# lazytiger/pbrt-rs

Hardware: AMD Instinct MI355X
Metric: Mrays/s (higher is better)
Workload: dtype f32

## Files before the change

pbrt-rs_amd/csrc/kernel_select.h:

```cpp
#pragma once
#include <type_traits>

#include "scene.h"
#include "trace_wide.h"

namespace pb {

enum class TraceKind { Stackless, Wide, Shapes, Spheres, Binary, Moving };
struct TraceChoice {
    TraceKind kind;
    int inst;
    bool count;
    bool ok;
};

inline TraceChoice choose_trace(const PbrtHipScene* s) {
    const PbrtHipContext* ctx = s->ctx;
    TraceChoice c{TraceKind::Binary, s->d.bvh.instanced ? (s->d.bvh.general_top ? 2 : 1) : 0, ctx->count_traversal == 1, true};
    if (ctx->traversal == PBRT_TRAVERSAL_STACKLESS) {
        c.kind = TraceKind::Stackless;
        c.ok = stackless_applies(s);
    } else if (s->has_wide && ctx->count_traversal != 1 && ctx->traversal == PBRT_TRAVERSAL_AUTO) {
        c.kind = TraceKind::Wide;
        c.count = ctx->count_traversal == 2;
// ... 78 lines not shown
                                               {k_shade_direct<D, 3>, k_shade_direct<W, 3>},
                                               {k_shade_direct<D, 2>, k_shade_direct<W, 2>},
                                               {k_shade_direct<D, 1>, k_shade_direct<W, 1>},
                                               {k_shade_direct<D, 0>, k_shade_direct<W, 0>}};
    static constexpr DirectKernel ao[2] = {k_shade_direct<AO, kDirectShapes>, k_shade_direct<AO, 0>};
    if (n.moving) return moving_direct_kernel(integrator);
    if (n.lobes && (integrator == D || integrator == W)) return lobe_direct_kernel(integrator == W);
    if (integrator == D || integrator == W) return lit[n.column()][integrator == W];
    return ao[n.shapes ? 0 : 1];
}

inline PathKernel path_kernel(const SceneNeeds& n, bool bin) {
    static constexpr PathKernel table[2][6] = {
        {k_shade_shapes<true>, k_shade_maps<true>, k_shade<true, 3>, k_shade<true, 2>, k_shade<true, 1>, k_shade<true, 0>},
        {k_shade_shapes<false>, k_shade_maps<false>, k_shade<false, 3>, k_shade<false, 2>, k_shade<false, 1>, k_shade<false, 0>}};
    if (n.moving) return moving_path_kernel(bin);
    if (n.lobes) return lobe_path_kernel(bin);
    return table[bin ? 0 : 1][n.column()];
}

inline DirectKernel lobe_direct_kernel(bool whitted) {
    static constexpr DirectKernel table[2] = {k_shade_direct<PBRT_INTEGRATOR_DIRECT, 3 + kDirectLobes>,
                                              k_shade_direct<PBRT_INTEGRATOR_WHITTED, 3 + kDirectLobes>};
    return table[whitted ? 1 : 0];
}
inline PathKernel lobe_path_kernel(bool bin) {
    static constexpr PathKernel table[2] = {k_shade_lobes<true>, k_shade_lobes<false>};
    return table[bin ? 0 : 1];
}

inline DirectKernel moving_direct_kernel(int integrator) {
    static constexpr DirectKernel table[3] = {k_shade_direct<PBRT_INTEGRATOR_DIRECT, 3 + kDirectMoving>,
                                              k_shade_direct<PBRT_INTEGRATOR_WHITTED, 3 + kDirectMoving>,
                                              k_shade_direct<PBRT_INTEGRATOR_AO, kDirectMoving>};
    return table[integrator == PBRT_INTEGRATOR_DIRECT ? 0 : integrator == PBRT_INTEGRATOR_WHITTED ? 1 : 2];
}
inline PathKernel moving_path_kernel(bool bin) {
    static constexpr PathKernel table[2] = {k_shade_moving<true>, k_shade_moving<false>};
    return table[bin ? 0 : 1];
}

using GenerateKernel = void (*)(PathState, Queues, PassParams, DevCamera, TileList);
using GenerateCameraKernel = void (*)(PathState, Queues, PassParams, DevCamera, DevMotion, TileList);
constexpr int kGenerateCameraAnimated = 2;
inline int generate_key(bool scene_moving, bool camera_animated) { return (scene_moving ? 1 : 0) | (camera_animated ? kGenerateCameraAnimated : 0); }
inline GenerateKernel generate_kernel(int key) {
    static constexpr GenerateKernel table[2] = {k_generate, k_generate_moving};
    return table[key & 1];
}
inline GenerateCameraKernel generate_camera_kernel(int key) {
    static constexpr GenerateCameraKernel table[2] = {k_generate_moving_camera, k_generate_moving_camera};
    return table[key & 1];
}
#endif

}
```

pbrt-rs_amd/csrc/render.hip:

```cpp
#include <hip/hip_runtime.h>
#include "abi_guard.h"

#include <algorithm>
#include <chrono>
#include <cstdio>
#include <cstdlib>
#include <cstring>
#include <string>
#include <thread>
#include <vector>

#include "host_motion.h"
#include "scene.h"
#include "trace.h"
#include "wavefront.h"
#define PB_SELECT_SHADING_KERNELS
#include "kernel_select.h"

using namespace pb;

static int camera_row(PbrtHipContext* ctx, const PbrtCamera& camera, const PbrtCameraMotion* motion, DevMotion* storage,
                      const DevMotion** row) {
    *row = nullptr;
    if (!motion || !motion->animated) return PBRT_HIP_OK;
// ... 777 lines not shown
        return hip_ok(ctx, hipEventCreate(&begin), "hipEventCreate") && hip_ok(ctx, hipEventCreate(&end), "hipEventCreate") &&
               hip_ok(ctx, hipEventCreate(&t0), "hipEventCreate") && hip_ok(ctx, hipEventCreate(&t1), "hipEventCreate");
    }
    ~RenderEvents() {
        for (hipEvent_t e : {begin, end, t0, t1})
            if (e) (void)hipEventDestroy(e);
    }
};

struct SortBufs {
    uint32_t *keys[2] = {nullptr, nullptr}, *vals = nullptr;
    void* tmp = nullptr;
    size_t tmp_bytes = 0;
};

constexpr int kSortFrom = 2;

struct RenderJob {
    PbrtHipScene* s;
    PbrtHipContext* ctx;
    hipStream_t st;
    const LiBatch* li;
    float* d_film;
    const DevMotion* camera_motion;
    PbrtRenderParams rp;
    bool li_mode, export_mode;
    bool tabulated;
    bool direct;
    bool box;
    float frx, fry;
    int32_t sb[4];
    int world, rank;
    int n_pix = 0, spp_pass = 0;
    int64_t valid_pixels = 0;
    size_t N = 0;
    PathState ps;
    Queues q[2];
    bool sort_rays = false, sort_shade = false, bin_shade = false;
    SortBufs ray_sort;
    SortBufs shade_sort;
    uint32_t* shade_positions = nullptr;
    TraceChoice trace;
    uint32_t* special_list = nullptr;
    std::vector<int> prefix;
    SamplerParams smp{};
    DirectState ds{};
    float* d_filter = nullptr;
    float4* accum = nullptr;
    TileList tiles{};
    DevCamera cam;
    ShadeConsts sc;
    DirectKernel shade_direct = nullptr;
    PathKernel shade_path[2] = {nullptr, nullptr};
    PbrtRenderStats local{};

    int invalid(const char* m) const {
        ctx->last_error = m;
        return PBRT_HIP_ERR_INVALID;
    }
    int round_count(int n) const { return rp.sampler == PBRT_SAMPLER_ZEROTWO ? round_up_pow2(n) : n; }
    const char* normalise_params(const PbrtRenderParams& rp_in);
    int size_pass();
    int alloc_path_buffers(DevBuf& buf, bool* ok);
    int setup_sampler(DevBuf& buf, bool* ok);
    int setup_light_distribution(const SceneNeeds& needs);
    PassParams pass_params(int s0) const;
    void wait_for_counts(int& rc);
    void trace_wavefront(const RenderEvents& ev, const Queues& qcur, uint32_t n_trace, int wavefront, int& rc);
    void shade_wavefront(const PassParams& pp, int cur, int nxt, uint32_t n_shade, int wavefront, int& rc);
    void run_wavefronts(const RenderEvents& ev, const PassParams& pp, uint32_t n_paths, int& rc);
    void film_stage(const PassParams& pp, uint32_t n_paths, bool last_pass, int& rc);
    int run(const PbrtCamera& camera, PbrtRenderStats* stats);
};

const char* RenderJob::normalise_params(const PbrtRenderParams& rp_in) {
    rp = rp_in;
    li_mode = li && li->d_rays;
    export_mode = li && li->out_rays;
    if (li_mode) {
        if (li->n <= 0 || li->n > (1ll << 28)) return "li: batch size must be in [1, 2^28]";
        rp.width = (int32_t)li->n;
        rp.height = 1;
        rp.spp = 1;
        rp.x0 = rp.y0 = 0;
        rp.x1 = rp.width;
        rp.y1 = 1;
        rp.tile_rank = 0;
        rp.tile_world = 1;
        rp.spp_per_pass = 1;
        rp.sampler = PBRT_SAMPLER_RANDOM;
        rp.filter_table = nullptr;
    }
    if (rp.width <= 0 || rp.height <= 0 || rp.spp <= 0) return "width, height and spp must be positive";
    if (rp.sampler < PBRT_SAMPLER_RANDOM || rp.sampler > PBRT_SAMPLER_HALTON) return "unknown sampler";
    tabulated = rp.sampler != PBRT_SAMPLER_RANDOM;
    if (tabulated && (rp.sampler_dims < 0 || rp.sampler_dims > 63)) return "sampler_dims must be in [0, 63]";
    if (const char* why = sampler_spp(rp, &rp.spp)) return why;
    if (rp.integrator == PBRT_INTEGRATOR_AO && rp.ao_samples >= 1 && rp.ao_samples <= 65535 && tabulated)
        rp.ao_samples = round_count(rp.ao_samples);
    frx = rp.filter_radius[0] > 0.0f ? rp.filter_radius[0] : 0.5f;
    fry = rp.filter_radius[1] > 0.0f ? rp.filter_radius[1] : 0.5f;
    box = true;
    if (rp.filter_table) {
        if (frx != 0.5f || fry != 0.5f) box = false;
        for (int i = 0; i < 256; ++i)
            if (rp.filter_table[i] != 1.0f) box = false;
// ... 204 lines not shown
    pp.n_pix = n_pix;
    pp.n_samples = std::min(spp_pass, rp.spp - s0);
    const int want = rp.samples_per_wave > 0 ? rp.samples_per_wave : ((tabulated && rp.sampler != PBRT_SAMPLER_HALTON) ? 1 : 64);
    pp.group_shift = 0;
    while ((2 << pp.group_shift) <= want && pp.group_shift < 6 && pp.n_samples % (2 << pp.group_shift) == 0) ++pp.group_shift;
    if (li_mode || export_mode) pp.group_shift = 0;
    pp.sample0 = s0;
    pp.spp = rp.spp;
    pp.width = rp.width;
    pp.height = rp.height;
    pp.x0 = rp.x0;
    pp.y0 = rp.y0;
    pp.x1 = rp.x1;
    pp.y1 = rp.y1;
    pp.sb_x0 = sb[0];
    pp.sb_y0 = sb[1];
    pp.sb_w = sb[2] - sb[0];
    pp.seed = rp.seed;
    pp.max_depth = rp.max_depth;
    pp.rr_threshold = rp.rr_threshold;
    pp.light_strategy = rp.light_strategy;
    pp.filter_rx = frx;
    pp.filter_ry = fry;
    pp.filter_table = d_filter;
    pp.max_sample_luminance = rp.max_sample_luminance > 0.0f ? rp.max_sample_luminance : INFINITY;
    pp.stream_keys = li_mode ? li->d_keys : nullptr;
    return pp;
}

#define RENDER_TRY(call) \
    if (rc == PBRT_HIP_OK && !hip_ok(ctx, (call), #call)) rc = PBRT_HIP_ERR_DEVICE;

void RenderJob::wait_for_counts(int& rc) {
    hipError_t qe;
    const auto spin_start = std::chrono::steady_clock::now();
    uint32_t polls = 0;
    while ((qe = hipEventQuery(ctx->ev_sync)) == hipErrorNotReady) {
        if ((++polls & 0xfffu) == 0) {
            const double waited = std::chrono::duration<double>(std::chrono::steady_clock::now() - spin_start).count();
            if (waited > ctx->wavefront_deadline_s) {
                ctx->last_error = "a wavefront did not finish within the deadline (hung kernel?)";
                ctx->lost = true;
                rc = PBRT_HIP_ERR_DEVICE;
                break;
            }
            if (waited > 0.05) std::this_thread::yield();
        }
    }
    if (rc == PBRT_HIP_OK) RENDER_TRY(qe);
}

void RenderJob::trace_wavefront(const RenderEvents& ev, const Queues& qcur, uint32_t n_trace, int wavefront, int& rc) {
    RENDER_TRY(hipMemsetAsync(ctx->d_work_counter, 0, kWorkCounters * sizeof(unsigned int), st));
    const uint32_t* trace_queue = qcur.trace;
    if (sort_rays && wavefront >= kSortFrom && n_trace >= (1u << 20)) {
        const SortBufs& rs = ray_sort;
        size_t tb = rs.tmp_bytes;
        if (pb::sort_pairs_u32(st, rs.tmp, &tb, rs.keys[0], rs.keys[1], qcur.trace, rs.vals, n_trace, kSortKeyBits) != 0 && rc == PBRT_HIP_OK) {
            ctx->last_error = "rocPRIM radix sort failed";
            rc = PBRT_HIP_ERR_DEVICE;
        }
        trace_queue = rs.vals;
    }
    RENDER_TRY(hipEventRecord(ev.t0, st));
    const int segments = (wavefront == 0 && !trace.inst) ? kQueueSegments : 1;
    dispatch(trace, [&](auto kind, auto count, auto inst) {
        constexpr TraceKind K = decltype(kind)::value;
        constexpr bool COUNT = decltype(count)::value;
        constexpr int INST = decltype(inst)::value;
        const dim3 grid(persistent_grid(s)), block(kTraceBlock);
        if constexpr (K == TraceKind::Stackless) {
            hipLaunchKernelGGL(k_trace_stackless, dim3(stackless_grid(s)), block, 0, st, s->d.bvh, ps, trace_queue, n_trace, ctx->d_work_counter,
                               segments);
        } else if constexpr (K == TraceKind::Wide) {
            WideTrees wt = s->wide;
            wt.special_list = special_list;
            wt.special_count = ctx->d_work_counter + kSpecialCount;
            hipLaunchKernelGGL((k_trace_wide<COUNT, INST>), dim3(wide_grid<COUNT, INST>(s)), block, 0, st, wt, ps, trace_queue, n_trace,
                               ctx->d_work_counter, segments, ctx->d_counters);
            hipLaunchKernelGGL(k_trace_special<INST>, grid, block, 0, st, s->d.bvh, ps, trace_queue, n_trace, special_list,
                               ctx->d_work_counter + kSpecialCount, ctx->d_work_counter + kFollowUpCounter);
        } else if constexpr (K == TraceKind::Shapes) {
            hipLaunchKernelGGL(k_trace_shapes<COUNT>, grid, block, 0, st, s->d.bvh, ps, trace_queue, n_trace, ctx->d_work_counter, ctx->d_counters,
                               segments);
        } else if constexpr (K == TraceKind::Moving) {
            hipLaunchKernelGGL((k_trace_moving<COUNT, INST>), dim3(persistent_grid(s, PB_MOVING_TRACE_WAVES)), block, 0, st, s->d.bvh, s->d_motions, ps,
                               trace_queue, n_trace, ctx->d_work_counter, ctx->d_counters, segments);
        } else {
            hipLaunchKernelGGL((k_trace<COUNT, INST, K == TraceKind::Spheres>), grid, block, 0, st, s->d.bvh, ps, trace_queue, n_trace,
                               ctx->d_work_counter, ctx->d_counters, segments);
        }
    });
    RENDER_TRY(hipGetLastError());
    RENDER_TRY(hipEventRecord(ev.t1, st));
}

void RenderJob::shade_wavefront(const PassParams& pp, int cur, int nxt, uint32_t n_shade, int wavefront, int& rc) {
    const dim3 grid((n_shade + 255) / 256), block(256);
    if (direct) {
        hipLaunchKernelGGL(shade_direct, grid, block, 0, st, sc, ps, ds, q[cur], q[nxt], pp, tiles, n_shade);
        return;
    }
    const Queues qin = q[cur];
    const uint32_t* order = nullptr;
    if (sort_shade && wavefront >= 1 && n_shade >= (1u << 10)) {
        const SortBufs& ss = shade_sort;
        hipLaunchKernelGGL(k_shade_sort_keys, dim3((n_shade + 255) / 256), dim3(256), 0, st, sc, ps, q[cur].shade, n_shade, pp.max_depth,
                           ss.keys[0], shade_positions);
        size_t tb = ss.tmp_bytes;
        if (pb::sort_pairs_u32(st, ss.tmp, &tb, ss.keys[0], ss.keys[1], shade_positions, ss.vals, n_shade, (s->bxdfs || s->disney || s->lobes) ? 4 : 3) != 0 &&
            rc == PBRT_HIP_OK) {
            ctx->last_error = "rocPRIM radix sort failed";
            rc = PBRT_HIP_ERR_DEVICE;
        }
        order = ss.vals;
    }
    hipLaunchKernelGGL(shade_path[bin_shade && wavefront >= 1], grid, block, 0, st, sc, ps, qin, q[nxt], pp, tiles, n_shade, order);
    std::swap(ps.ray, ps.ray_next);
    std::swap(ps.nee_a, ps.nee_a_next);
    std::swap(ps.nee_f, ps.nee_f_next);
    std::swap(ps.nee_b, ps.nee_b_next);
    std::swap(ps.nee_light, ps.nee_light_next);
}

void RenderJob::run_wavefronts(const RenderEvents& ev, const PassParams& pp, uint32_t n_paths, int& rc) {
    unsigned long long counts[2] = {n_paths, n_paths};
    local.camera_samples += (uint64_t)valid_pixels * pp.n_samples;
    local.rays_closest += (uint64_t)valid_pixels * pp.n_samples;
    int cur = 0, wavefront = 0;
    while (rc == PBRT_HIP_OK && counts[1] > 0) {
        uint32_t n_trace = (uint32_t)counts[0], n_shade = (uint32_t)counts[1];
        if (n_trace > 0) trace_wavefront(ev, q[cur], n_trace, wavefront, rc);
        int nxt = cur ^ 1;
        RENDER_TRY(hipMemsetAsync(q[nxt].counts64, 0, 2 * sizeof(unsigned long long), st));
        q[nxt].keys = (sort_rays && wavefront + 1 >= kSortFrom) ? ray_sort.keys[0] : nullptr;
        shade_wavefront(pp, cur, nxt, n_shade, wavefront, rc);
        RENDER_TRY(hipGetLastError());
        RENDER_TRY(hipMemcpyAsync(ctx->h_counts, q[nxt].counts64, sizeof(counts), hipMemcpyDeviceToHost, st));
        RENDER_TRY(hipEventRecord(ctx->ev_sync, st));
        if (rc == PBRT_HIP_OK) wait_for_counts(rc);
        counts[0] = ctx->h_counts[0];
        counts[1] = ctx->h_counts[1];
        if (n_trace > 0 && rc == PBRT_HIP_OK) {
            float ms = 0.0f;
            RENDER_TRY(hipEventElapsedTime(&ms, ev.t0, ev.t1));
            local.trace_ms += ms;
            local.trace_launches += 1;
            if (ctx->trace_log)
                std::fprintf(stderr, "[pbrt_hip] k_trace: %u rays %.3f ms (%.0f Mrays/s), k_shade: %u paths\n", n_trace, ms, n_trace / ms * 1e-3,
                             n_shade);
            ctx->trace_ms += ms;
            ctx->trace_launches += 1;
        }
        const uint64_t n_rays = counts[0] & 0xffffffffull, n_shadow = counts[0] >> 32;
        local.rays_closest += n_rays - n_shadow;
        local.rays_shadow += n_shadow;
        counts[0] = n_rays;
        wavefront += 1;
        cur = nxt;
    }
}

void RenderJob::film_stage(const PassParams& pp, uint32_t n_paths, bool last_pass, int& rc) {
    if (li_mode) {
        hipLaunchKernelGGL(k_li_output, dim3((unsigned)((li->n + 255) / 256)), dim3(256), 0, st, ps, (uint32_t)li->n, li->d_rgb);
        RENDER_TRY(hipGetLastError());
        return;
    }
    if (!box) {
        hipLaunchKernelGGL(k_film_splat, dim3((n_paths + 255) / 256), dim3(256), 0, st, ps, pp, tiles, d_film);
// ... 35 lines not shown
        valid_pixels += (int64_t)(std::min(o.x + kTile, rp.x1) - o.x) * (std::min(o.y + kTile, rp.y1) - o.y);
    if (li_mode) valid_pixels = li->n;
    if (int rc = size_pass()) return rc;
    if (export_mode && spp_pass != rp.spp) return invalid("camera rays: too many samples for one pass");
    N = (size_t)n_pix * spp_pass;
    if (N * 4 >= (1ull << 32)) return invalid("too many concurrent paths for 32-bit queue entries; lower spp_per_pass");

    DevBuf buf(ctx);
    bool ok = true;
    if (int rc = alloc_path_buffers(buf, &ok)) return rc;
    if (int rc = setup_sampler(buf, &ok)) return rc;
    int* d_prefix = buf.alloc<int>(prefix.size(), &ok);
    if (direct) {
        ds.stage = buf.alloc<int>(N, &ok);
        ds.ld_acc = buf.alloc<float4>(N, &ok);
        ds.frames = buf.alloc<float4>(N * (size_t)std::max(1, rp.max_depth) * 3, &ok);
        ds.light_strategy = rp.light_strategy;
        ds.mode = rp.integrator;
        ds.ao_samples = rp.ao_samples;
        ds.ao_cos_sample = rp.light_strategy != 0;
        if (prefix.back() >= 0xfff0) return invalid("too many light samples per vertex");
    }
    if (!box) {
        d_filter = buf.alloc<float>(256, &ok);
        if (ok) HIP_TRY(ctx, hipMemcpyAsync(d_filter, rp.filter_table, 256 * sizeof(float), hipMemcpyHostToDevice, st));
    }
    accum = buf.alloc<float4>(n_pix, &ok);
    int2* d_origins = buf.alloc<int2>(origins.size(), &ok);
    if (!ok) return PBRT_HIP_ERR_OOM;
    HIP_TRY(ctx, hipMemcpyAsync(d_origins, origins.data(), origins.size() * sizeof(int2), hipMemcpyHostToDevice, st));
    HIP_TRY(ctx, hipMemsetAsync(accum, 0, (size_t)n_pix * sizeof(float4), st));
    HIP_TRY(ctx, hipMemcpyAsync(d_prefix, prefix.data(), prefix.size() * sizeof(int), hipMemcpyHostToDevice, st));
    tiles = TileList{d_origins, (int)origins.size()};

    std::memcpy(cam.c2w, camera.camera_to_world, 64);
    std::memcpy(cam.r2c, camera.raster_to_camera, 64);
    cam.lens_radius = camera.lens_radius;
    cam.focal_distance = camera.focal_distance;
    cam.shutter_open = camera.shutter_open;
    cam.shutter_close = camera.shutter_close;
    cam.kind = camera.kind;
    if (camera.kind < PBRT_CAMERA_PERSPECTIVE || camera.kind > PBRT_CAMERA_ENVIRONMENT) return invalid("unknown camera kind");

    const SceneNeeds needs = scene_needs(s);
    scene_shade_consts(s, &sc);
    sc.light_sample_prefix = d_prefix;
    sc.total_light_samples = prefix.back();
    if (int rc = setup_light_distribution(needs)) return rc;
    if (direct) {
        shade_direct = direct_kernel(needs, rp.integrator);
    } else {
        shade_path[0] = path_kernel(needs, false);
        shade_path[1] = path_kernel(needs, true);
    }

    RenderEvents ev;
    if (!ev.create(ctx)) return PBRT_HIP_ERR_DEVICE;
    int rc = PBRT_HIP_OK;
    RENDER_TRY(hipEventRecord(ev.begin, st));
    bool tables_ready = !tabulated || rp.sampler == PBRT_SAMPLER_HALTON;
    for (int s0 = 0; s0 < rp.spp && rc == PBRT_HIP_OK; s0 += spp_pass) {
        const PassParams pp = pass_params(s0);
        const uint32_t n_paths = (uint32_t)n_pix * pp.n_samples;
        if (!tables_ready) {
            hipLaunchKernelGGL(k_sampler_tables, dim3((n_pix + 63) / 64), dim3(64), 0, st, pp, tiles);
            RENDER_TRY(hipGetLastError());
            tables_ready = true;
        }
        if (li_mode)
            hipLaunchKernelGGL(k_li_generate, dim3((n_paths + 255) / 256), dim3(256), 0, st, ps, q[0], li->d_rays, li->d_keys, (uint32_t)li->n,
                               n_paths, li->skip);
        else if (const int key = generate_key(s->moving, camera_motion != nullptr); key & kGenerateCameraAnimated)
            hipLaunchKernelGGL(generate_camera_kernel(key), dim3((n_paths + 255) / 256), dim3(256), 0, st, ps, q[0], pp, cam, *camera_motion, tiles);
        else
            hipLaunchKernelGGL(generate_kernel(key), dim3((n_paths + 255) / 256), dim3(256), 0, st, ps, q[0], pp, cam, tiles);
        RENDER_TRY(hipGetLastError());
        if (export_mode) {
            hipLaunchKernelGGL(k_camera_rays_out, dim3((n_paths + 255) / 256), dim3(256), 0, st, ps, pp, tiles, li->out_rays, li->out_keys,
                               li->out_pfilm, li->out_pixel_sample);
            RENDER_TRY(hipGetLastError());
            break;
        }
        if (direct) {
            RENDER_TRY(hipMemsetAsync(ds.stage, 0, (size_t)n_paths * sizeof(int), st));
            RENDER_TRY(hipMemsetAsync(ds.ld_acc, 0, (size_t)n_paths * sizeof(float4), st));
        }
        run_wavefronts(ev, pp, n_paths, rc);
        film_stage(pp, n_paths, s0 + spp_pass >= rp.spp, rc);
    }
    RENDER_TRY(hipEventRecord(ev.end, st));
    if (!ctx->lost) {
        const hipError_t drained = hipStreamSynchronize(st);
        if (rc == PBRT_HIP_OK && !hip_ok(ctx, drained, "hipStreamSynchronize (end of render)")) rc = PBRT_HIP_ERR_DEVICE;
    }
    if (rc == PBRT_HIP_OK) {
        float ms = 0.0f;
        RENDER_TRY(hipEventElapsedTime(&ms, ev.begin, ev.end));
        local.total_ms = ms;
    }
    if (stats) *stats = local;
    return rc;
}
}

int wavefront_render(PbrtHipScene* s, const PbrtCamera& camera, const PbrtRenderParams& rp_in, float* d_film,
                     PbrtRenderStats* stats, const LiBatch* li, const DevMotion* camera_motion) {
    RenderJob job{s, s->ctx, s->ctx->stream, li, d_film, camera_motion};
    if (const char* why = job.normalise_params(rp_in)) return job.invalid(why);
    return job.run(camera, stats);
}
#undef RENDER_TRY

#ifdef PB_LANE_STATS
extern "C" int pbrt_hip_debug_wide_stats(unsigned long long* out24, int reset) try {
    if (hipMemcpyFromSymbol(out24, HIP_SYMBOL(pb::g_wide_stats), 32 * sizeof(unsigned long long)) != hipSuccess) return 1;
    if (reset) {
        unsigned long long z[32] = {0};
        if (hipMemcpyToSymbol(HIP_SYMBOL(pb::g_wide_stats), z, sizeof(z)) != hipSuccess) return 1;
    }
    return 0;
}
PB_ABI_CATCH
extern "C" int pbrt_hip_debug_lane_stats(unsigned long long* out8, int reset) try {
    if (hipMemcpyFromSymbol(out8, HIP_SYMBOL(pb::g_lane_stats), 8 * sizeof(unsigned long long)) != hipSuccess) return 1;
    if (reset) {
        unsigned long long z[8] = {0, 0, 0, 0, 0, 0, 0, 0};
        if (hipMemcpyToSymbol(HIP_SYMBOL(pb::g_lane_stats), z, sizeof(z)) != hipSuccess) return 1;
    }
// ... 5 lines not shown
```

pbrt-rs_amd/csrc/wavefront.h:

```cpp
#pragma once
#include <hip/hip_runtime.h>

#include "wf_state.h"
#include "wf_sampler.h"
#include "wf_generate_trace.h"
#include "wf_surface.h"
#include "wf_lights.h"
#include "wf_lobes.h"
#include "wf_path.h"
#include "wf_direct.h"
#include "wf_film.h"
#include "wf_camera_motion.h"

struct LiBatch {
    const PbrtRay* d_rays = nullptr;
    const uint64_t* d_keys = nullptr;
    int64_t n = 0;
    int skip = 0;
    float* d_rgb = nullptr;
    PbrtRay* out_rays = nullptr;
    uint64_t* out_keys = nullptr;
    float* out_pfilm = nullptr;
    int32_t* out_pixel_sample = nullptr;
};
int wavefront_render(PbrtHipScene* s, const PbrtCamera& camera, const PbrtRenderParams& rp, float* d_film,
                     PbrtRenderStats* stats, const LiBatch* li = nullptr, const pb::DevMotion* camera_motion = nullptr);
```

pbrt-rs_amd/csrc/wf_generate_trace.h:

```cpp
#pragma once
#include "wf_sampler.h"

namespace pb {

PB_DEV void camera_rows_at(const DevCamera& cam, const DevMotion& mo, float time, float* rows) {
    if (time <= mo.start_time) {
        for (int k = 0; k < 12; ++k) rows[k] = cam.c2w[k];
    } else if (time >= mo.end_time) {
        for (int k = 0; k < 12; ++k) rows[k] = mo.end_o2w[k];
    } else {
        motion_interpolate_forward(mo, time, rows);
    }
}
PB_DEV V3 xform_point_rows(const float* m, V3 p) {
    return V3{m[0] * p.x + m[1] * p.y + m[2] * p.z + m[3], m[4] * p.x + m[5] * p.y + m[6] * p.z + m[7],
              m[8] * p.x + m[9] * p.y + m[10] * p.z + m[11]};
}

template <bool TIME, bool CAMERA_MOTION = false>
PB_DEV void generate_camera_rays(const PathState& ps, const Queues& q, const PassParams& pp, const DevCamera& cam, const TileList& tiles,
                                 const DevMotion* cmo = nullptr) {
    uint32_t p = blockIdx.x * blockDim.x + threadIdx.x;
    uint32_t n = (uint32_t)pp.n_pix * pp.n_samples;
    if (p >= n) return;
    int s_local, pix;
    path_to_sample_pixel(pp, p, &s_local, &pix);
    int tile = pix >> 8, within = pix & 255;
    int2 org = tiles.origin[tile];
    int x = org.x + (within & 15), y = org.y + (within >> 4);
    bool valid = x >= pp.x0 && x < pp.x1 && y >= pp.y0 && y < pp.y1;
    int flags = 0;
    if (valid) {
        int s = pp.sample0 + s_local;
        Samp sm;
        rng_set_sequence(sm.rng, sample_sequence(pp, x, y, s));
        sm.pix = pix;
        sm.s = s;
        sm.dim1 = sm.dim2 = sm.arr = 0;
        sm.h_offset = pp.smp.kind == PBRT_SAMPLER_HALTON ? halton_pixel_offset(pp.smp, x, y) : 0;
        float u0, u1, l0, l1;
        samp_2d(pp, sm, &u0, &u1);
        float pfx = (float)x + u0, pfy = (float)y + u1;
        float time_u = samp_1d(pp, sm);
        samp_2d(pp, sm, &l0, &l1);
        V3 o = V3{0.0f, 0.0f, 0.0f}, d;
        if (cam.kind == PBRT_CAMERA_ENVIRONMENT) {
            float theta = kPi * pfy / (float)pp.height;
            float phi = 2.0f * kPi * pfx / (float)pp.width;
            float st, ct, sp, cp;
            det_sincos(theta, &st, &ct);
            det_sincos(phi, &sp, &cp);
            d = V3{st * cp, ct, st * sp};
        } else if (cam.kind == PBRT_CAMERA_ORTHOGRAPHIC) {
            o = xform_point(cam.r2c, V3{pfx, pfy, 0.0f});
            d = V3{0.0f, 0.0f, 1.0f};
            if (cam.lens_radius > 0.0f) {
                float lx, ly;
                concentric_sample_disk(l0, l1, &lx, &ly);
                lx *= cam.lens_radius;
                ly *= cam.lens_radius;
                float ft = cam.focal_distance / d.z;
                V3 p_focus = o + d * ft;
                o.x += lx;
                o.y += ly;
                d = normalize(p_focus - o);
            }
        } else {
            V3 p_camera = xform_point(cam.r2c, V3{pfx, pfy, 0.0f});
            d = normalize(p_camera);
            if (cam.lens_radius > 0.0f) {
                float lx, ly;
                concentric_sample_disk(l0, l1, &lx, &ly);
                lx *= cam.lens_radius;
                ly *= cam.lens_radius;
                float ft = cam.focal_distance / d.z;
                V3 p_focus = o + d * ft;
                o = V3{lx, ly, 0.0f};
                d = normalize(p_focus - o);
            }
        }
        (void)time_u;
        const float* m = cam.c2w;
        float rows[12], time = 0.0f;
        if (CAMERA_MOTION) {
            time = (1.0f - time_u) * cam.shutter_open + time_u * cam.shutter_close;
            camera_rows_at(cam, *cmo, time, rows);
            m = rows;
        }
        V3 ow = CAMERA_MOTION ? xform_point_rows(m, o) : xform_point(m, o);
        float xa = __builtin_fabsf(m[0] * o.x) + __builtin_fabsf(m[1] * o.y) + __builtin_fabsf(m[2] * o.z) + __builtin_fabsf(m[3]);
        float ya = __builtin_fabsf(m[4] * o.x) + __builtin_fabsf(m[5] * o.y) + __builtin_fabsf(m[6] * o.z) + __builtin_fabsf(m[7]);
        float za = __builtin_fabsf(m[8] * o.x) + __builtin_fabsf(m[9] * o.y) + __builtin_fabsf(m[10] * o.z) + __builtin_fabsf(m[11]);
        V3 o_err = V3{xa, ya, za} * kGamma3;
        V3 dw = xform_vector(m, d);
        float l2 = len2(dw);
        float tmax = kInf;
        if (l2 > 0.0f) {
            float dt = dot(vabs(dw), o_err) / l2;
            ow = ow + dw * dt;
            tmax -= dt;
        }
        store_ray(ps, p, RS_CONT, ow, dw, tmax);
        if (CAMERA_MOTION)
            ps.ray[ray_index(ps, p, RS_CONT) + 1].w = time;
        else if (TIME)
            ps.ray[ray_index(ps, p, RS_CONT) + 1].w = (1.0f - time_u) * cam.shutter_open + time_u * cam.shutter_close;
        samp_store(ps, p, sm);
        ps.pfilm[p] = make_float2(pfx, pfy);
        flags = PF_VALID | PF_ALIVE;
    } else {
        ps.pfilm[p] = make_float2(0.0f, 0.0f);
    }
    ps.L[p] = make_float4(0.0f, 0.0f, 0.0f, 1.0f);
    ps.beta[p] = make_float4(1.0f, 1.0f, 1.0f, __int_as_float(flags));
    if (!valid) store_ray(ps, p, RS_CONT, V3{0.0f, 0.0f, 0.0f}, V3{0.0f, 0.0f, 1.0f}, -1.0f);
    q.trace[p] = p * 4u + RS_CONT;
    q.shade[p] = p;
}
__global__ void k_generate(PathState ps, Queues q, PassParams pp, DevCamera cam, TileList tiles) {
    generate_camera_rays<false>(ps, q, pp, cam, tiles);
}

__global__ void k_li_generate(PathState ps, Queues q, const PbrtRay* __restrict__ rays, const uint64_t* __restrict__ keys, uint32_t n,
                              uint32_t n_padded, int skip) {
    uint32_t p = blockIdx.x * blockDim.x + threadIdx.x;
    if (p >= n_padded) return;
    int flags = 0;
    if (p < n) {
        Rng rng;
        rng_set_sequence(rng, keys[p]);
        for (int k = 0; k < skip; ++k) (void)rng_u32(rng);
        ps.rng[p] = rng.state;
        ps.samp[p] = 0;
        const float4* rp = reinterpret_cast<const float4*>(rays + p);
        float4 a = rp[0], b = rp[1];
        store_ray(ps, p, RS_CONT, V3{a.x, a.y, a.z}, V3{a.w, b.x, b.y}, b.z);
        ps.ray[ray_index(ps, p, RS_CONT) + 1].w = b.w;
        flags = PF_VALID | PF_ALIVE;
    } else {
        store_ray(ps, p, RS_CONT, V3{0.0f, 0.0f, 0.0f}, V3{0.0f, 0.0f, 1.0f}, -1.0f);
    }
    ps.pfilm[p] = make_float2(0.0f, 0.0f);
    ps.L[p] = make_float4(0.0f, 0.0f, 0.0f, 1.0f);
    ps.beta[p] = make_float4(1.0f, 1.0f, 1.0f, __int_as_float(flags));
    q.trace[p] = p * 4u + RS_CONT;
    q.shade[p] = p;
}
__global__ void k_li_output(PathState ps, uint32_t n, float* __restrict__ rgb) {
    uint32_t p = blockIdx.x * blockDim.x + threadIdx.x;
    if (p >= n) return;
    float4 L = ps.L[p];
    rgb[3 * (size_t)p] = L.x;
    rgb[3 * (size_t)p + 1] = L.y;
    rgb[3 * (size_t)p + 2] = L.z;
}
__global__ void k_camera_rays_out(PathState ps, PassParams pp, TileList tiles, PbrtRay* __restrict__ rays, uint64_t* __restrict__ keys,
                                  float* __restrict__ pfilm, int32_t* __restrict__ pixel_sample) {
    uint32_t p = blockIdx.x * blockDim.x + threadIdx.x;
    uint32_t n = (uint32_t)pp.n_pix * pp.n_samples;
    if (p >= n) return;
    int s_local, pix;
    path_to_sample_pixel(pp, p, &s_local, &pix);
    int2 org = tiles.origin[pix >> 8];
    int x = org.x + (pix & 15), y = org.y + ((pix & 255) >> 4);
    bool valid = (__float_as_int(ps.beta[p].w) & PF_VALID) != 0;
    size_t ri = ray_index(ps, p, RS_CONT);
    float4 a = ps.ray[ri], b = ps.ray[ri + 1];
    float4* out = reinterpret_cast<float4*>(rays + p);
    out[0] = a;
    out[1] = b;
    keys[p] = sample_sequence(pp, x, y, pp.sample0 + s_local);
    float2 pf = ps.pfilm[p];
    pfilm[2 * (size_t)p] = pf.x;
    pfilm[2 * (size_t)p + 1] = pf.y;
    pixel_sample[3 * (size_t)p] = valid ? x : -1;
    pixel_sample[3 * (size_t)p + 1] = valid ? y : -1;
    pixel_sample[3 * (size_t)p + 2] = pp.sample0 + s_local;
}

template <bool TWO_LEVEL>
struct WavefrontRayIO {
    PathState ps;
    const uint32_t* __restrict__ queue;
    uint32_t count;
    int n_segments;
    PB_DEV uint32_t n() const { return count; }
    PB_DEV int segments() const { return n_segments; }
    PB_DEV uint32_t token(uint32_t i) const { return queue[i]; }
    PB_DEV bool strict(uint32_t e) const { return (e & 3u) == RS_MIS_BOOL; }
    PB_DEV bool load(uint32_t e, TravRay* r, bool* any) const {
        uint32_t p = e >> 2, slot = e & 3u;
        size_t ri = ray_index(ps, p, slot == RS_MIS_BOOL ? (uint32_t)RS_MIS : slot);
        float4 a = ps.ray[ri], b = ps.ray[ri + 1];
        *r = TravRay{a.x, a.y, a.z, a.w, b.x, b.y, b.z};
        *any = slot >= RS_SHADOW;
        return !(b.z < 0.0f);
    }
    PB_DEV bool load(uint32_t e, TravRay* r, bool* any, float* time) const {
        uint32_t p = e >> 2, slot = e & 3u;
        size_t ri = ray_index(ps, p, slot == RS_MIS_BOOL ? (uint32_t)RS_MIS : slot);
        float4 a = ps.ray[ri], b = ps.ray[ri + 1];
        *r = TravRay{a.x, a.y, a.z, a.w, b.x, b.y, b.z};
        *any = slot >= RS_SHADOW;
        *time = b.w;
        return !(b.z < 0.0f);
    }
    PB_DEV void store(uint32_t e, bool any, bool found, float t, float b0, float b1, float b2, int slot, int inst) const {
        uint32_t p = e >> 2, rs = e & 3u;
        if (rs == RS_MIS_BOOL) {
            ps.hit[hit_index(ps, p, RS_MIS)] = make_float4(__int_as_float(found ? 0 : -1), 0.0f, 0.0f, 0.0f);
            return;
        }
        size_t ri = hit_index(ps, p, rs);
        if (any) {
            ps.hit[ri] = make_float4(found ? 1.0f : 0.0f, 0.0f, 0.0f, 0.0f);
        } else {
            (void)t;
            ps.hit[ri] = make_float4(__int_as_float(found ? slot : -1), b0, b1, b2);
            if (TWO_LEVEL) ps.hit[ri + 1] = make_float4(__int_as_float(inst), 0.0f, 0.0f, 0.0f);
        }
    }
};

template <bool COUNT, int INST, bool SPH = false>
__global__ void __launch_bounds__(kTraceBlock, (COUNT || SPH) ? 4 : (INST ? PB_INST_WAVES : PB_TRACE_WAVES))
    k_trace(DevBVH bvh, PathState ps, const uint32_t* __restrict__ queue, uint32_t n, unsigned int* work_counter,
            unsigned long long* counters, int segments) {
    __shared__ uint2 lds_stack[kStackLds * kTraceBlock];
    WavefrontRayIO<INST != 0> io{ps, queue, n, segments};
    trace_persistent<WavefrontRayIO<INST != 0>, COUNT, INST, SPH>(bvh, io, work_counter, lds_stack + threadIdx.x,
                                                  blockIdx.x * kTraceBlock + threadIdx.x, counters);
}

template <bool COUNT>
__global__ void __launch_bounds__(kTraceBlock, 4)
    k_trace_shapes(DevBVH bvh, PathState ps, const uint32_t* __restrict__ queue, uint32_t n, unsigned int* work_counter,
                   unsigned long long* counters, int segments) {
    __shared__ uint2 lds_stack[kStackLds * kTraceBlock];
    WavefrontRayIO<false> io{ps, queue, n, segments};
    trace_persistent<WavefrontRayIO<false>, COUNT, 0, false, true>(bvh, io, work_counter, lds_stack + threadIdx.x,
                                                                   blockIdx.x * kTraceBlock + threadIdx.x, counters);
// ... 47 lines not shown
```

pbrt-rs_amd/csrc/wf_path.h:

```cpp
#pragma once
#include "wf_lights.h"

namespace pb {

PB_DEV uint32_t shade_key(const ShadeConsts& sc, const PathState& ps, uint32_t p, uint32_t rec, int max_depth) {
    int fb = __float_as_int(ps.beta[p].w);
    uint32_t key = 0;
    if ((fb & PF_ALIVE) && (fb >> 8) < max_depth) {
        const size_t hb = hit_index(ps, rec, RS_CONT);
        int slot = __float_as_int(ps.hit[hb].x), inst = hit_instance(ps, hb);
        if (slot >= 0) {
            int mat = __float_as_int(sc.bvh.tris[3 * (size_t)slot + 2].z);
            if (sc.bvh.instanced && inst >= 0) {
                int over = __float_as_int(sc.bvh.instances[7 * (size_t)inst + 6].x);
                if (over >= 0) mat = over;
            }
            key = 1u + (uint32_t)sc.materials[mat].type;
        }
    }
    return key;
}
__global__ void k_shade_sort_keys(ShadeConsts sc, PathState ps, const uint32_t* __restrict__ shade_queue, uint32_t n, int max_depth,
                                  uint32_t* __restrict__ keys, uint32_t* __restrict__ positions) {
    uint32_t i = blockIdx.x * blockDim.x + threadIdx.x;
    if (i >= n) return;
    keys[i] = shade_key(sc, ps, shade_queue[i], i, max_depth);
    positions[i] = i;
}

constexpr int shade_keys(int level) { return level == 4 ? 13 : level == 3 ? 12 : level == 2 ? 11 : level == 1 ? 8 : 6; }
template <int KEYS>
struct ShadeBins {
    uint32_t count[4][KEYS];
    uint32_t path[256];
    uint32_t rec[256];
};

#ifndef PB_SHADE_WAVES
#define PB_SHADE_WAVES 3
#endif
template <bool BIN, int LEVEL, bool SHP, bool ML = false, bool MOV = false>
PB_DEV void shade_bounce(const ShadeConsts& sc, const PathState& ps, const Queues& qin, const Queues& qout, const PassParams& pp,
                         const TileList& tiles, uint32_t n_in, const uint32_t* __restrict__ order) {
    constexpr bool GLOSSY = LEVEL >= 1;
    constexpr bool LOBES = LEVEL == 4;
    constexpr int kShadeKeys = shade_keys(LEVEL);
    uint32_t i = blockIdx.x * blockDim.x + threadIdx.x;
    bool active = i < n_in;
    uint32_t rec = (active && order) ? order[i] : i;
    uint32_t p = active ? qin.shade[rec] : 0u;
    __shared__ StagedRecords staged;
    const StageSink stage{staged};
    if (BIN) {
        __shared__ ShadeBins<kShadeKeys> bins;
        const int lane = threadIdx.x & 63, wave = threadIdx.x >> 6;
        const uint32_t key = active ? shade_key(sc, ps, p, rec, pp.max_depth) : (uint32_t)(kShadeKeys - 1);
        uint32_t rank = 0;
#pragma unroll
        for (int k = 0; k < kShadeKeys; ++k) {
            const unsigned long long m = __ballot(key == (uint32_t)k);
            if (key == (uint32_t)k) rank = lane_prefix(m);
            if (lane == 0) bins.count[wave][k] = (uint32_t)__popcll(m);
        }
        __syncthreads();
        uint32_t before = 0;
        for (int k = 0; k < kShadeKeys; ++k)
            for (int w = 0; w < 4; ++w)
                before += ((uint32_t)k < key || ((uint32_t)k == key && w < wave)) ? bins.count[w][k] : 0u;
        bins.path[before + rank] = p;
        bins.rec[before + rank] = rec;
        uint32_t n_active = 0;
        for (int k = 0; k < kShadeKeys - 1; ++k)
            for (int w = 0; w < 4; ++w) n_active += bins.count[w][k];
        __syncthreads();
        p = bins.path[threadIdx.x];
        rec = bins.rec[threadIdx.x];
        active = threadIdx.x < n_active;
    }
    bool emit_cont = false, emit_mis = false, emit_shadow = false, mis_bool = false;

    uint32_t cell = 0;
    float time = 0.0f;
    if (active) {
        float4 Lq = ps.L[p], bq = ps.beta[p];
        V3 L = V3{Lq.x, Lq.y, Lq.z};
        float eta_scale = Lq.w;
        V3 beta = V3{bq.x, bq.y, bq.z};
        int fb = __float_as_int(bq.w);
        int flags = fb & 0xff, bounces = fb >> 8;
        size_t rbase = ray_index(ps, rec, RS_CONT), hbase = hit_index(ps, rec, RS_CONT);

        if (flags & (PF_NEE_SHADOW | PF_NEE_MIS)) {
            float pick_pdf;
            V3 beta_v;
            V3 ld = estimate_direct_resolve<SHP>(sc, ps, rec, flags, &pick_pdf, &beta_v);
            ld = ld / pick_pdf;
            L = L + mulv(beta_v, ld);
            flags &= ~(PF_NEE_SHADOW | PF_NEE_MIS);
        }

        if (flags & PF_ALIVE) {
            flags &= ~PF_ALIVE;
            float4 r0 = ps.ray[rbase], r1 = ps.ray[rbase + 1];
            V3 rd = V3{r0.w, r1.x, r1.y};
            float4 h0 = ps.hit[hbase];
            int hslot = __float_as_int(h0.x);
            bool found = hslot >= 0;
            Surf sf;
            if (MOV) time = r1.w;
            if (found) {
                if constexpr (MOV)
                    sf = surface_from_hit_moving(sc.bvh, sc.motions, time, hslot, hit_instance(ps, hbase), h0.y, h0.z, h0.w, rd);
                else
                    sf = surface_from_hit<SHP>(sc.bvh, hslot, hit_instance(ps, hbase), h0.y, h0.z, h0.w, rd);
                if (qout.keys) cell = ray_sort_cell(sf.p.x, sf.p.y, sf.p.z, qout.key_lo, qout.key_inv);
            }
            if (bounces == 0 || (flags & PF_SPECULAR_BOUNCE)) {
                if (found) {
                    L = L + mulv(beta, surface_le(sc, sf, -rd));
                } else {
                    for (int k = 0; k < sc.n_infinite; ++k) {
                        DevLight lt = sc.lights[sc.infinite_ids[k]];
                        V3 le = lt.slot >= 0 ? env_le(sc.env_maps[lt.slot], rd) : V3{lt.L[0], lt.L[1], lt.L[2]};
                        L = L + mulv(beta, le);
                    }
                }
            }
            if (found && bounces < pp.max_depth) {
                DevMaterial mat = sc.materials[sf.material];
                Samp sm = path_sampler(ps, pp, tiles, p);
                if (mat.type == PBRT_MAT_NONE) {
                    V3 o = offset_ray_origin(sf.p, sf.p_error, sf.n, rd);
                    stage.ray(RS_CONT, o, rd, kInf);
                    flags |= PF_ALIVE;
                    emit_cont = true;
                } else {
                    Frame fr = make_frame(sf);
                    V3 kd = V3{mat.kd[0], mat.kd[1], mat.kd[2]};
                    V3 kt = V3{mat.kt[0], mat.kt[1], mat.kt[2]};
                    V3 wo = -rd;
                    bool has_lobe;
                    bool nonspecular;
                    typename LevelBsdf<LEVEL>::type nsb;
                    if (GLOSSY) {
                        load_bsdf(sc, sf.material, mat, &nsb);
                        nonspecular = nsb.n > 0;
                        if (mat.type == PBRT_MAT_GLASS) has_lobe = !(is_black(kd) && is_black(kt));
                        else if (mat.type == PBRT_MAT_MIRROR) has_lobe = !is_black(kd);
                        else has_lobe = nonspecular;
                        if constexpr (LOBES)
                            if (nsb.row) has_lobe = nsb.row->n > 0;
                    } else {
                        if (mat.type == PBRT_MAT_GLASS) has_lobe = !(is_black(kd) && is_black(kt));
                        else has_lobe = !is_black(kd);
                        nonspecular = (mat.type == PBRT_MAT_MATTE) && has_lobe;
                    }
// ... 128 lines not shown
```

Measured before the change: 3026.

## Use implicit identity queues and initial path state for the first wavefront

```diff
diff --git a/pbrt-rs_amd/csrc/kernel_select.h b/pbrt-rs_amd/csrc/kernel_select.h
--- a/pbrt-rs_amd/csrc/kernel_select.h
+++ b/pbrt-rs_amd/csrc/kernel_select.h
@@ -154,6 +154,22 @@
     static constexpr GenerateCameraKernel table[2] = {k_generate_moving_camera, k_generate_moving_camera};
     return table[key & 1];
 }
+
+inline GenerateKernel implicit_generate_kernel(int key) {
+    static constexpr GenerateKernel table[2] = {k_generate_implicit, k_generate_moving_implicit};
+    return table[key & 1];
+}
+inline GenerateCameraKernel implicit_generate_camera_kernel(int key) {
+    static constexpr GenerateCameraKernel table[2] = {k_generate_moving_camera_implicit, k_generate_moving_camera_implicit};
+    return table[key & 1];
+}
+inline PathKernel first_path_kernel(const SceneNeeds& n) {
+    static constexpr PathKernel table[6] = {k_shade_shapes_first, k_shade_maps_first, k_shade_first<3>,
+                                            k_shade_first<2>,     k_shade_first<1>,   k_shade_first<0>};
+    if (n.moving) return k_shade_moving_first;
+    if (n.lobes) return k_shade_lobes_first;
+    return table[n.column()];
+}
 #endif
 
 }
diff --git a/pbrt-rs_amd/csrc/render.hip b/pbrt-rs_amd/csrc/render.hip
--- a/pbrt-rs_amd/csrc/render.hip
+++ b/pbrt-rs_amd/csrc/render.hip
@@ -853,6 +853,8 @@
     ShadeConsts sc;
     DirectKernel shade_direct = nullptr;
     PathKernel shade_path[2] = {nullptr, nullptr};
+    PathKernel shade_first = nullptr;
+    bool implicit_gen0 = false;
     PbrtRenderStats local{};
 
     int invalid(const char* m) const {
@@ -1163,7 +1165,7 @@
 
 void RenderJob::trace_wavefront(const RenderEvents& ev, const Queues& qcur, uint32_t n_trace, int wavefront, int& rc) {
     RENDER_TRY(hipMemsetAsync(ctx->d_work_counter, 0, kWorkCounters * sizeof(unsigned int), st));
-    const uint32_t* trace_queue = qcur.trace;
+    const uint32_t* trace_queue = (implicit_gen0 && wavefront == 0) ? nullptr : qcur.trace;
     if (sort_rays && wavefront >= kSortFrom && n_trace >= (1u << 20)) {
         const SortBufs& rs = ray_sort;
         size_t tb = rs.tmp_bytes;
@@ -1226,7 +1228,8 @@
         }
         order = ss.vals;
     }
-    hipLaunchKernelGGL(shade_path[bin_shade && wavefront >= 1], grid, block, 0, st, sc, ps, qin, q[nxt], pp, tiles, n_shade, order);
+    const PathKernel kernel = (implicit_gen0 && wavefront == 0) ? shade_first : shade_path[bin_shade && wavefront >= 1];
+    hipLaunchKernelGGL(kernel, grid, block, 0, st, sc, ps, qin, q[nxt], pp, tiles, n_shade, order);
     std::swap(ps.ray, ps.ray_next);
     std::swap(ps.nee_a, ps.nee_a_next);
     std::swap(ps.nee_f, ps.nee_f_next);
@@ -1368,6 +1371,8 @@
     } else {
         shade_path[0] = path_kernel(needs, false);
         shade_path[1] = path_kernel(needs, true);
+        shade_first = first_path_kernel(needs);
+        implicit_gen0 = !li_mode && !export_mode;
     }
 
     RenderEvents ev;
@@ -1387,9 +1392,11 @@
             hipLaunchKernelGGL(k_li_generate, dim3((n_paths + 255) / 256), dim3(256), 0, st, ps, q[0], li->d_rays, li->d_keys, (uint32_t)li->n,
                                n_paths, li->skip);
         else if (const int key = generate_key(s->moving, camera_motion != nullptr); key & kGenerateCameraAnimated)
-            hipLaunchKernelGGL(generate_camera_kernel(key), dim3((n_paths + 255) / 256), dim3(256), 0, st, ps, q[0], pp, cam, *camera_motion, tiles);
+            hipLaunchKernelGGL(implicit_gen0 ? implicit_generate_camera_kernel(key) : generate_camera_kernel(key), dim3((n_paths + 255) / 256),
+                               dim3(256), 0, st, ps, q[0], pp, cam, *camera_motion, tiles);
         else
-            hipLaunchKernelGGL(generate_kernel(key), dim3((n_paths + 255) / 256), dim3(256), 0, st, ps, q[0], pp, cam, tiles);
+            hipLaunchKernelGGL(implicit_gen0 ? implicit_generate_kernel(key) : generate_kernel(key), dim3((n_paths + 255) / 256), dim3(256), 0, st,
+                               ps, q[0], pp, cam, tiles);
         RENDER_TRY(hipGetLastError());
         if (export_mode) {
             hipLaunchKernelGGL(k_camera_rays_out, dim3((n_paths + 255) / 256), dim3(256), 0, st, ps, pp, tiles, li->out_rays, li->out_keys,
diff --git a/pbrt-rs_amd/csrc/wavefront.h b/pbrt-rs_amd/csrc/wavefront.h
--- a/pbrt-rs_amd/csrc/wavefront.h
+++ b/pbrt-rs_amd/csrc/wavefront.h
@@ -11,6 +11,7 @@
 #include "wf_direct.h"
 #include "wf_film.h"
 #include "wf_camera_motion.h"
+#include "wf_gen0.h"
 
 struct LiBatch {
     const PbrtRay* d_rays = nullptr;
diff --git a/pbrt-rs_amd/csrc/wf_gen0.h b/pbrt-rs_amd/csrc/wf_gen0.h
--- /dev/null
+++ b/pbrt-rs_amd/csrc/wf_gen0.h
@@ -0,0 +1,38 @@
+#pragma once
+#include "wf_camera_motion.h"
+
+namespace pb {
+
+__global__ void k_generate_implicit(PathState ps, Queues q, PassParams pp, DevCamera cam, TileList tiles) {
+    generate_camera_rays<false, false, true>(ps, q, pp, cam, tiles);
+}
+__global__ void k_generate_moving_implicit(PathState ps, Queues q, PassParams pp, DevCamera cam, TileList tiles) {
+    generate_camera_rays<true, false, true>(ps, q, pp, cam, tiles);
+}
+__global__ void k_generate_moving_camera_implicit(PathState ps, Queues q, PassParams pp, DevCamera cam, DevMotion cmo, TileList tiles) {
+    generate_camera_rays<true, true, true>(ps, q, pp, cam, tiles, &cmo);
+}
+
+template <int LEVEL>
+__global__ void __launch_bounds__(256, LEVEL == 3 ? 2 : PB_SHADE_WAVES) k_shade_first(ShadeConsts sc, PathState ps, Queues qin, Queues qout, PassParams pp,
+                                                       TileList tiles, uint32_t n_in, const uint32_t* __restrict__ order) {
+    shade_bounce<false, LEVEL, false, false, false, true>(sc, ps, qin, qout, pp, tiles, n_in, order);
+}
+__global__ void __launch_bounds__(256, 2) k_shade_shapes_first(ShadeConsts sc, PathState ps, Queues qin, Queues qout, PassParams pp,
+                                                              TileList tiles, uint32_t n_in, const uint32_t* __restrict__ order) {
+    shade_bounce<false, 3, true, true, false, true>(sc, ps, qin, qout, pp, tiles, n_in, order);
+}
+__global__ void __launch_bounds__(256, 2) k_shade_maps_first(ShadeConsts sc, PathState ps, Queues qin, Queues qout, PassParams pp,
+                                                            TileList tiles, uint32_t n_in, const uint32_t* __restrict__ order) {
+    shade_bounce<false, 3, false, true, false, true>(sc, ps, qin, qout, pp, tiles, n_in, order);
+}
+__global__ void __launch_bounds__(256, 2) k_shade_lobes_first(ShadeConsts sc, PathState ps, Queues qin, Queues qout, PassParams pp,
+                                                             TileList tiles, uint32_t n_in, const uint32_t* __restrict__ order) {
+    shade_bounce<false, 4, false, false, false, true>(sc, ps, qin, qout, pp, tiles, n_in, order);
+}
+__global__ void __launch_bounds__(256, 2) k_shade_moving_first(ShadeConsts sc, PathState ps, Queues qin, Queues qout, PassParams pp,
+                                                              TileList tiles, uint32_t n_in, const uint32_t* __restrict__ order) {
+    shade_bounce<false, 3, false, false, true, true>(sc, ps, qin, qout, pp, tiles, n_in, order);
+}
+
+}
diff --git a/pbrt-rs_amd/csrc/wf_generate_trace.h b/pbrt-rs_amd/csrc/wf_generate_trace.h
--- a/pbrt-rs_amd/csrc/wf_generate_trace.h
+++ b/pbrt-rs_amd/csrc/wf_generate_trace.h
@@ -17,7 +17,7 @@
               m[8] * p.x + m[9] * p.y + m[10] * p.z + m[11]};
 }
 
-template <bool TIME, bool CAMERA_MOTION = false>
+template <bool TIME, bool CAMERA_MOTION = false, bool IMPLICIT = false>
 PB_DEV void generate_camera_rays(const PathState& ps, const Queues& q, const PassParams& pp, const DevCamera& cam, const TileList& tiles,
                                  const DevMotion* cmo = nullptr) {
     uint32_t p = blockIdx.x * blockDim.x + threadIdx.x;
@@ -111,11 +111,15 @@
     } else {
         ps.pfilm[p] = make_float2(0.0f, 0.0f);
     }
-    ps.L[p] = make_float4(0.0f, 0.0f, 0.0f, 1.0f);
-    ps.beta[p] = make_float4(1.0f, 1.0f, 1.0f, __int_as_float(flags));
+    if (!IMPLICIT) {
+        ps.L[p] = make_float4(0.0f, 0.0f, 0.0f, 1.0f);
+        ps.beta[p] = make_float4(1.0f, 1.0f, 1.0f, __int_as_float(flags));
+    }
     if (!valid) store_ray(ps, p, RS_CONT, V3{0.0f, 0.0f, 0.0f}, V3{0.0f, 0.0f, 1.0f}, -1.0f);
-    q.trace[p] = p * 4u + RS_CONT;
-    q.shade[p] = p;
+    if (!IMPLICIT) {
+        q.trace[p] = p * 4u + RS_CONT;
+        q.shade[p] = p;
+    }
 }
 __global__ void k_generate(PathState ps, Queues q, PassParams pp, DevCamera cam, TileList tiles) {
     generate_camera_rays<false>(ps, q, pp, cam, tiles);
@@ -186,7 +190,7 @@
     int n_segments;
     PB_DEV uint32_t n() const { return count; }
     PB_DEV int segments() const { return n_segments; }
-    PB_DEV uint32_t token(uint32_t i) const { return queue[i]; }
+    PB_DEV uint32_t token(uint32_t i) const { return queue ? queue[i] : i << 2; }
     PB_DEV bool strict(uint32_t e) const { return (e & 3u) == RS_MIS_BOOL; }
     PB_DEV bool load(uint32_t e, TravRay* r, bool* any) const {
         uint32_t p = e >> 2, slot = e & 3u;
diff --git a/pbrt-rs_amd/csrc/wf_path.h b/pbrt-rs_amd/csrc/wf_path.h
--- a/pbrt-rs_amd/csrc/wf_path.h
+++ b/pbrt-rs_amd/csrc/wf_path.h
@@ -39,16 +39,17 @@
 #ifndef PB_SHADE_WAVES
 #define PB_SHADE_WAVES 3
 #endif
-template <bool BIN, int LEVEL, bool SHP, bool ML = false, bool MOV = false>
+template <bool BIN, int LEVEL, bool SHP, bool ML = false, bool MOV = false, bool FIRST = false>
 PB_DEV void shade_bounce(const ShadeConsts& sc, const PathState& ps, const Queues& qin, const Queues& qout, const PassParams& pp,
                          const TileList& tiles, uint32_t n_in, const uint32_t* __restrict__ order) {
     constexpr bool GLOSSY = LEVEL >= 1;
     constexpr bool LOBES = LEVEL == 4;
     constexpr int kShadeKeys = shade_keys(LEVEL);
+    static_assert(!(FIRST && BIN), "the first launch is never binned");
     uint32_t i = blockIdx.x * blockDim.x + threadIdx.x;
     bool active = i < n_in;
-    uint32_t rec = (active && order) ? order[i] : i;
-    uint32_t p = active ? qin.shade[rec] : 0u;
+    uint32_t rec = (!FIRST && active && order) ? order[i] : i;
+    uint32_t p = FIRST ? (active ? i : 0u) : active ? qin.shade[rec] : 0u;
     __shared__ StagedRecords staged;
     const StageSink stage{staged};
     if (BIN) {
@@ -82,15 +83,26 @@
     uint32_t cell = 0;
     float time = 0.0f;
     if (active) {
-        float4 Lq = ps.L[p], bq = ps.beta[p];
-        V3 L = V3{Lq.x, Lq.y, Lq.z};
-        float eta_scale = Lq.w;
-        V3 beta = V3{bq.x, bq.y, bq.z};
-        int fb = __float_as_int(bq.w);
-        int flags = fb & 0xff, bounces = fb >> 8;
         size_t rbase = ray_index(ps, rec, RS_CONT), hbase = hit_index(ps, rec, RS_CONT);
-
-        if (flags & (PF_NEE_SHADOW | PF_NEE_MIS)) {
+        V3 L = V3{0.0f, 0.0f, 0.0f}, beta = V3{1.0f, 1.0f, 1.0f};
+        float eta_scale = 1.0f;
+        int flags, bounces = 0;
+        float4 r0, r1;
+        if (FIRST) {
+            r0 = ps.ray[rbase];
+            r1 = ps.ray[rbase + 1];
+            flags = r1.z < 0.0f ? 0 : (PF_ALIVE | PF_VALID);
+        } else {
+            float4 Lq = ps.L[p], bq = ps.beta[p];
+            L = V3{Lq.x, Lq.y, Lq.z};
+            eta_scale = Lq.w;
+            beta = V3{bq.x, bq.y, bq.z};
+            int fb = __float_as_int(bq.w);
+            flags = fb & 0xff;
+            bounces = fb >> 8;
+        }
+
+        if (!FIRST && (flags & (PF_NEE_SHADOW | PF_NEE_MIS))) {
             float pick_pdf;
             V3 beta_v;
             V3 ld = estimate_direct_resolve<SHP>(sc, ps, rec, flags, &pick_pdf, &beta_v);
@@ -101,7 +113,10 @@
 
         if (flags & PF_ALIVE) {
             flags &= ~PF_ALIVE;
-            float4 r0 = ps.ray[rbase], r1 = ps.ray[rbase + 1];
+            if (!FIRST) {
+                r0 = ps.ray[rbase];
+                r1 = ps.ray[rbase + 1];
+            }
             V3 rd = V3{r0.w, r1.x, r1.y};
             float4 h0 = ps.hit[hbase];
             int hslot = __float_as_int(h0.x);
```

After: 3026, median of 2. No clear change (-0.0%).
